# pandegroup/openmm

Hardware: NVIDIA H100
Metric: ns/day (higher is better)
Workload: dtype f32

## Files before the change

openmm_b200/csrc/engine.cu:

```cuda
#include "engine.h"
#include "../../include/b200md.h"
#include <stdexcept>
#include <algorithm>
#include <cmath>
#include <cstring>
#include <cstdlib>
#include <map>
#include <set>
#include <dlfcn.h>
#include <thread>

static std::string g_create_error;

template <class T> struct DevBuf {
    T* p = nullptr; size_t n = 0; bool owned = true;
    void attach(void* ptr, size_t count) { free(); p = (T*) ptr; n = count; owned = false; }
    void alloc(size_t count) {
        if (!owned) { if (count > n) throw std::runtime_error("window buffer too small"); return; }
        free(); n = count; if (count) CUDA_CHECK(cudaMalloc(&p, count*sizeof(T)));
    }
    void upload(const std::vector<T>& v) { if (v.size() > n) alloc(v.size()); if (!v.empty()) CUDA_CHECK(cudaMemcpy(p, v.data(), v.size()*sizeof(T), cudaMemcpyHostToDevice)); }
    void zero() { if (n) CUDA_CHECK(cudaMemset(p, 0, n*sizeof(T))); }
    void free() { if (p && owned) cudaFree(p); p = nullptr; n = 0; owned = true; }
    ~DevBuf() { free(); }
// ... 58 lines not shown
struct b200md_ctx {
    int device = 0;
    int natoms = 0, npad = 0, nblocks = 0;
    bool finalized = false;
    std::string err;
    cudaStream_t stream = nullptr;
    cudaStream_t streamPme = nullptr;
    cudaStream_t streamBonded = nullptr;
    cudaEvent_t evFork = nullptr, evJoin = nullptr, evJoinBonded = nullptr, evForkGrid = nullptr;
    bool pmeOnly = false;
    bool listDirty = true;
    bool overlapPme = true;
    bool pmeBrick = true;
    int brickAtoms = 64, brickPoints = 8192;
    bool listBuilt = false;
    std::vector<double> mass, charge, sigma, epsilon;
    b200md_nonbonded_desc nbdesc{};
    bool haveNb = false;
    struct { std::vector<int2> atoms; std::vector<double3> params; DevBuf<int2> atomsDev; DevBuf<double4> paramsDev; } exc;
    TermTable<int2, double2> bonds;
    TermTable<int4, double2> angles;
    TermTable<int4, double4> torsions;
    TermTable<int4, double> rb;
    CmapTable cmap;
    std::vector<int> conI, conJ; std::vector<double> conD;
    int cmFreq = 0;
    std::vector<int4> hUnitAtoms;
    double boxA[3] = {0, 0, 0}, boxB[3] = {0, 0, 0}, boxC[3] = {0, 0, 0};
    bool haveBox = false;
    bool haveOrigin = false;
    double padFrac = 0.10;
    DevBuf<float4> posq, velm, sposq[2], swrap[2], refPos, atomShift, blockCenter[2], blockHalf[2], superCenter[2], superHalf[2];
    DevBuf<float2> sigeps, ssigeps[2];
    DevBuf<double> chargeD; DevBuf<double2> sigepsD;
    DevBuf<long long> force;
    DevBuf<double> energy, cmScratch;
    DevBuf<int> molStart, molAtoms, cellOffset, sorig[2], sortedOf, cellRank, cellCount, cellFill, atomCell, tmpSorted, tileI[2], tileJ[2], tileMask[2], listCounters, counters, exclStart, exclList;
    DevBuf<unsigned int> maskPool[2];
    DevBuf<unsigned long long> stepCounter;
    DevBuf<unsigned int> blocksDone;
    bool stepStateValid = false;
    DevBuf<real> grid, eterm;
    DevBuf<long long> gridFixed;
    DevBuf<real2> cgrid;
    DevBuf<real2> tw[3];
    DevBuf<double> moduli[3];
    DevBuf<int4> unitAtoms; DevBuf<int> unitType; DevBuf<float4> unitParams;
    std::vector<int> ccmaCons;
    DevBuf<int> ccCompCon, ccCompAtom, ccRowStart, ccCol, ccAtoms, ccAStart, ccACon;
    DevBuf<int2> ccConAtoms; DevBuf<float> ccDist, ccRedMass, ccVal, ccDelta1, ccDelta2;
    DevBuf<float4> ccRij, ccXold, ccXunc;
    int precision = B200MD_PRECISION_SINGLE;
    DevBuf<float4> posqCorr; DevBuf<double4> velmD, unitParamsD;
    DevBuf<double> ccDistD, ccRedMassD, ccDelta1D, ccDelta2D; DevBuf<double4> ccRijD, ccXoldD, ccXuncD, ccXposD;
    bool mixed() const { return precision == B200MD_PRECISION_MIXED; }
    CcmaDev ccma{};
    NbDev nb{};
    PmeDev pme{};
    BondedDev bd{};
    UnitDev units{};
    IntegDev integ{};
    bool haveIntegrator = false;
    double dt = 0, temperature = 0, friction = 0;
    double time = 0;
    int64_t stepCount = 0;
    double selfEnergy = 0, dispersionCoefficient = 0;
    int64_t forceEvals = 0, kernelLaunches = 0, graphInstantiations = 0;
    DevBuf<int> baroStart, baroAtoms;
// ... 882 lines not shown
extern "C" int b200md_finalize(b200md_ctx* ctx) {
    API_BEGIN(ctx)
    require(!ctx->finalized, "finalize called twice");
    b200md_ctx* c = ctx;
    const int N = c->natoms, NP = c->npad;
    if (!c->haveNb) { c->nbdesc = b200md_nonbonded_desc{}; c->nbdesc.method = B200MD_NB_NOCUTOFF; }
    NbDev& nb = c->nb;
    nb.natoms = N; nb.npad = NP; nb.nblocks = c->nblocks;
    nb.method = c->nbdesc.method;
    nb.rank = c->rank; nb.world = c->world;
    c->cd = CommDev{}; c->cd.world = 1;
    c->p2p = c->world > 1 && c->comm && !(getenv("B200MD_MGPU") && std::string(getenv("B200MD_MGPU")) == "nccl");
    if (c->p2p) setup_window(c);
    { const double cc = getenv("B200MD_CLOSE_NM") ? atof(getenv("B200MD_CLOSE_NM")) : 0.36; nb.closeCut2 = (float) (cc*cc); }
    for (int w = 0; w < 4; w++) nb.pmeSmMask[w] = 0ull;
    nb.smPartition = false;
    if (c->nbdesc.method == B200MD_NB_PME && !c->pmeOnly && c->overlapPme) {
        int want = 0;
        if (c->p2p) want = std::min(74, std::max((c->nbdesc.grid[0] + c->world - 1)/c->world, 16 + 6*c->world));
        if (getenv("B200MD_PME_SMS")) want = atoi(getenv("B200MD_PME_SMS"));
        const int got = want > 0 ? choose_pme_sms(want, nb.pmeSmMask) : 0;
        if (got > 0) {
            nb.smPartition = true;
            const int planes = (c->nbdesc.grid[0] + c->world - 1)/c->world;
            fft_set_compact(planes > got ? 2 : 1);
        }
    }
    c->posq.alloc(NP); c->posq.zero(); c->velm.alloc(NP); c->velm.zero();
    c->refPos.alloc(NP); c->refPos.zero(); c->atomShift.alloc(NP); c->sigeps.alloc(NP);
    c->listCounters.alloc(2*LC_STRIDE); c->listCounters.zero();
    for (int l = 0; l < 2; l++) {
        c->sposq[l].alloc(NP); c->sposq[l].zero(); c->swrap[l].alloc(NP); c->swrap[l].zero(); c->ssigeps[l].alloc(NP); c->ssigeps[l].zero();
        c->sorig[l].alloc(NP); c->sorig[l].zero(); c->blockCenter[l].alloc(c->nblocks); c->blockHalf[l].alloc(c->nblocks);
        ListDev& L = c->nb.list[l];
        L.sposq = c->sposq[l].p; L.ssigeps = c->ssigeps[l].p; L.swrap = c->swrap[l].p; L.sorig = c->sorig[l].p;
        c->superCenter[l].alloc((c->nblocks + 31)/32); c->superHalf[l].alloc((c->nblocks + 31)/32);
        L.superCenter = c->superCenter[l].p; L.superHalf = c->superHalf[l].p;
        L.blockCenter = c->blockCenter[l].p; L.blockHalf = c->blockHalf[l].p; L.lc = c->listCounters.p + LC_STRIDE*l;
    }
    c->force.alloc((size_t) 3*NP); c->force.zero();
    c->energy.alloc(B200MD_NUM_ENERGY); c->energy.zero(); c->cmScratch.alloc(12); c->cmScratch.zero();
    c->blocksDone.alloc(1); c->blocksDone.zero();
    c->sortedOf.alloc(NP); c->atomCell.alloc(NP); c->tmpSorted.alloc(NP);
    c->counters.alloc(16); c->counters.zero();
    c->stepCounter.alloc(1); c->stepCounter.zero();
    std::vector<float4> vm(NP, make_float4(0, 0, 0, 0));
    for (int i = 0; i < N; i++) vm[i].w = (c->mass[i] > 0) ? (float) (1.0/c->mass[i]) : 0.f;
    c->velm.upload(vm);
    nb.posqCorr = nullptr; nb.velmD = nullptr;
    if (c->mixed()) {
        std::vector<double4> vd(NP, make_double4(0, 0, 0, 0));
        for (int i = 0; i < N; i++) vd[i].w = (c->mass[i] > 0) ? 1.0/c->mass[i] : 0.0;
        c->posqCorr.alloc(NP); c->posqCorr.zero(); c->velmD.upload(vd);
        nb.posqCorr = c->posqCorr.p; nb.velmD = c->velmD.p;
    }
    nb.posq = c->posq.p; nb.velm = c->velm.p; nb.sigeps = c->sigeps.p; nb.force = c->force.p; nb.energy = c->energy.p;
    nb.sortedOf = c->sortedOf.p;
    nb.refPos = c->refPos.p; nb.atomCell = c->atomCell.p; nb.tmpSorted = c->tmpSorted.p; nb.atomShift = c->atomShift.p;
    nb.counters = c->counters.p;
    const double rc = c->nbdesc.cutoff;
    if (nb.method == B200MD_NB_NOCUTOFF) {
        nb.cutoff = 1e18f; nb.cutoff2 = 3e38f; nb.paddedCutoff2 = 3e38f; nb.halfPad2 = 3e38f;
    }
    else {
        const double pad = c->padFrac*rc;
        nb.cutoff = (float) rc; nb.cutoff2 = (float) (rc*rc); nb.paddedCutoff2 = (float) ((rc+pad)*(rc+pad)); nb.halfPad2 = (float) (0.25*pad*pad);
    }
    nb.useSwitch = c->nbdesc.use_switch; nb.switchDist = (float) c->nbdesc.switch_distance;
    nb.alpha = (float) c->nbdesc.ewald_alpha;
    if (nb.method == B200MD_NB_CUTOFF_PERIODIC || nb.method == B200MD_NB_CUTOFF_NONPERIODIC) {
        const double eps = c->nbdesc.rf_dielectric;
        nb.krf = (float) (std::pow(rc, -3.0)*(eps-1.0)/(2.0*eps+1.0));
        nb.crf = (float) ((1.0/rc)*(3.0*eps)/(2.0*eps+1.0));
    }
    {
        std::vector<std::vector<int> > ex(N);
        for (const int2& a : c->exc.atoms) { ex[a.x].push_back(a.y); ex[a.y].push_back(a.x); }
        std::vector<int> start(N+1, 0), list;
        for (int i = 0; i < N; i++) {
            std::sort(ex[i].begin(), ex[i].end());
            ex[i].erase(std::unique(ex[i].begin(), ex[i].end()), ex[i].end());
            start[i+1] = start[i] + (int) ex[i].size();
            list.insert(list.end(), ex[i].begin(), ex[i].end());
        }
        if (list.empty()) list.push_back(0);
        c->exclStart.upload(start); c->exclList.upload(list);
        nb.exclStart = c->exclStart.p; nb.exclList = c->exclList.p;
    }
    alloc_tile_pools(c, initial_pool_capacity(c));
// ... 357 lines not shown
            launch_pme_spread(c->nb, pme, c->cd, sp, !forkAfterList); launches++;
            if (p2p) { launch_grid_push(c->pme, c->cd, sp); launches++; }
            else if (c->world > 1 && c->comm && !split) {
                int rc = g_nccl.AllReduce(c->gridFixed.p, c->gridFixed.p, (size_t) c->pme.nx*c->pme.ny*c->pme.nz, NCCL_INT64, NCCL_SUM, c->comm, sp);
                if (rc != 0) throw std::runtime_error("ncclAllReduce(grid) failed");
            }
            launch_pme_fft_conv(c->nb, c->pme, c->cd, energy && (split || p2p || c->rank == 0), fft_beside_tiles(c), sp); launches += pme_fft_launch_count(c->pme);
            launch_pme_gather(c->nb, pme, c->cd, sp); launches++;
        }
        if (fork) CUDA_CHECK(cudaEventRecord(c->evJoin, sp));
    };
    if (!forkAfterList) launch_recip();
    if (forkAfterList && recip) {
        CUDA_CHECK(cudaEventRecord(c->evForkGrid, s));
        CUDA_CHECK(cudaStreamWaitEvent(sp, c->evForkGrid, 0));
        CUDA_CHECK(cudaMemsetAsync(pme.gridFixed, 0, sizeof(long long)*(size_t) pme.nx*pme.ny*pme.nz, sp));
    }
    if (direct) {
        launch_check_displacement(c->nb, c->cd, s); launches++;
        launch_list_build(c->nb, s); launches += LIST_BUILD_LAUNCHES;
    }
    int bterms = terms & (B200MD_TERM_BONDS | B200MD_TERM_ANGLES | B200MD_TERM_TORSIONS | B200MD_TERM_RB_TORSIONS | B200MD_TERM_CMAP);
    if (c->haveNb) bterms |= terms & B200MD_TERM_NB_DIRECT;
    const int nbonded = c->bd.nbonds + c->bd.nangles + c->bd.ntorsions + c->bd.nrb + c->bd.ncmap + c->bd.nexc;
    const bool bonded = bterms && nbonded > 0 && !(split && c->rank == pmeRank);
    auto launch_bonded_terms = [&](cudaStream_t sb) { BondedDev bd = c->bd; bd.groupMask = groupMask; launch_bonded(c->nb, bd, bterms, energy, sb); launches++; };
    const bool forkBonded = forkAfterList && bonded;
    if (forkAfterList) launch_recip();
    if (forkBonded) {
        CUDA_CHECK(cudaStreamWaitEvent(c->streamBonded, c->evFork, 0));
        launch_bonded_terms(c->streamBonded);
        CUDA_CHECK(cudaEventRecord(c->evJoinBonded, c->streamBonded));
    }
    if (direct) { launch_pair(c->nb, energy, s); launches++; }
    if (bonded && !forkBonded) launch_bonded_terms(s);
    const bool pushEarly = p2p && fork;
    if (pushEarly) { launch_force_push(c->nb, c->cd, s); launches++; }
    if (fork) CUDA_CHECK(cudaStreamWaitEvent(s, c->evJoin, 0));
    if (forkBonded) CUDA_CHECK(cudaStreamWaitEvent(s, c->evJoinBonded, 0));
    if (p2p) {
        if (!pushEarly) { launch_force_push(c->nb, c->cd, s); launches++; }
        if (!inStep) { launch_force_total(c->nb, c->cd, s); launches += 2; }
    }
    if (c->world > 1 && c->comm) {
        int rc = 0;
        if (!p2p) rc = g_nccl.AllReduce(c->force.p, c->force.p, (size_t) 3*c->npad, NCCL_INT64, NCCL_SUM, c->comm, s);
        if (rc != 0) throw std::runtime_error("ncclAllReduce(force) failed");
        if (energy) {
            rc = g_nccl.AllReduce(c->energy.p, c->energy.p, B200MD_NUM_ENERGY, NCCL_FLOAT64, NCCL_SUM, c->comm, s);
            if (rc != 0) throw std::runtime_error("ncclAllReduce(energy) failed");
        }
    }
    CUDA_CHECK(cudaGetLastError());
    return launches;
}

static void check_flags(b200md_ctx* c) {
    if (!c->finalized) return;
    int h[8];
    CUDA_CHECK(cudaMemcpyAsync(h, c->counters.p, sizeof(int)*8, cudaMemcpyDeviceToHost, c->stream));
    CUDA_CHECK(cudaStreamSynchronize(c->stream));
    if (h[CT_OVERFLOW] == 2) throw std::runtime_error("B200 platform: neighbour-list construction timed out at a grid barrier (k_list_prep)");
    if (h[CT_OVERFLOW] == 3) throw std::runtime_error("B200 platform: multi-GPU exchange timed out waiting for a peer rank (every rank must issue the same sequence of calls)");
    if (h[CT_OVERFLOW]) throw std::runtime_error("B200 platform: neighbour-list tile capacity exceeded (" + std::to_string(c->nb.maxTiles) + " tiles) during the preceding steps; the trajectory since the last state read is invalid");
}

static bool role_split(const b200md_ctx* c);
// ... 404 lines not shown
```

openmm_b200/csrc/engine.h:

```cpp
#pragma once
#include <cuda_runtime.h>
#include <stdint.h>
#include <stdexcept>
#include <string>
#include <vector>

#define B200MD_TILE 32
#define B200MD_PME_ORDER 5
#define B200MD_FORCE_SCALE 4294967296.0
#define B200MD_ONE_4PI_EPS0 138.93545764438198
#define B200MD_BOLTZ 0.00831446261815324
#define B200MD_MAX_RADIX 16
#define B200MD_MAX_FFT_STAGES 8

#define CUDA_CHECK(x) do { cudaError_t e_ = (x); if (e_ != cudaSuccess) throw std::runtime_error(std::string(#x) + ": " + cudaGetErrorString(e_)); } while (0)

template <typename... P, typename... A>
inline void launch_high(void (*kernel)(P...), dim3 grid, dim3 block, size_t smem, cudaStream_t s, A... args) {
    static const int hi = [] { int lo = 0, h = 0; cudaDeviceGetStreamPriorityRange(&lo, &h); return h; }();
    cudaLaunchAttribute at[1];
    at[0].id = cudaLaunchAttributePriority;
    at[0].val.priority = hi;
    cudaLaunchConfig_t cfg = {};
    cfg.gridDim = grid; cfg.blockDim = block; cfg.dynamicSmemBytes = smem; cfg.stream = s;
    cfg.attrs = at; cfg.numAttrs = 1;
    CUDA_CHECK(cudaLaunchKernelEx(&cfg, kernel, args...));
}

struct BoxDev {
    float ax, bx, by, cx, cy, cz;
    float invAx, invBy, invCz;
    int triclinic;
    int periodic;
    double dax, dby, dcz;
    double recip[9];
    double volume;
};

#ifdef B200MD_REAL_DOUBLE
typedef double real;
typedef double2 real2;
#else
typedef float real;
typedef float2 real2;
#endif

struct FftPlanDev {
    int n;
    int nstages;
    int radix[B200MD_MAX_FFT_STAGES];
    const real2* tw;
};

struct ListDev {
    float4* sposq;
    float2* ssigeps;
    float4* swrap;
    int* sorig;
    float4* blockCenter;
    float4* blockHalf;
    float4* superCenter;
    float4* superHalf;
    int* tileI;
    int* tileJ;
    int* tileMask;
    unsigned int* maskPool;
    int* lc;
};
#define TILE_REGIONS 32
enum { LC_TILES = 0, LC_MASKS = TILE_REGIONS, LC_MAXHALF = 2*TILE_REGIONS, LC_USED = 2*TILE_REGIONS + 1, LC_STRIDE = 128 };

enum { CT_PAIRSTART = 0,
       CT_REBUILD = 2, CT_OVERFLOW = 3, CT_BUILDS = 4, CT_PAIRS = 5, CT_CUR = 10, CT_CURSOR = 14,
       CT_BTDONE = 7, CT_BAR = 9, CT_BAREXIT = 15 };

struct NbDev {
    BoxDev box;
    int natoms, npad, nblocks;
    int method;
    int useSwitch;
    float cutoff, cutoff2, paddedCutoff2, switchDist;
    float alpha;
    float krf, crf;
    float dispDummy;
    float4* posq;
    float4* velm;
    float4* posqCorr;
    double4* velmD;
    float2* sigeps;
    const double* chargeD;
    const double2* sigepsD;
    long long* force;
    double* energy;
    ListDev list[2];
    int* sortedOf;
    float4* refPos;
    int ncell[3];
    int ncells;
    const int* cellRank;
    int* cellCount;
    int* cellFill;
    int* atomCell;
    int* tmpSorted;
    float4* atomShift;
    int maxTiles;
    int* counters;
    const int* exclStart;
    const int* exclList;
    int nmol;
    const int* molStart;
    const int* molAtoms;
    int* cellOffset;
    float halfPad2;
    int rank, world;
    double origin[3];
    unsigned long long pmeSmMask[4];
    bool smPartition;
    float closeCut2;
};

enum { EN_NB = 0, EN_RECIP = 1, EN_BOND = 2, EN_ANGLE = 3, EN_TORSION = 4, EN_EXC = 5, EN_KE = 6, EN_RBTORSION = 7, EN_CMAP = 8,
       B200MD_NUM_ENERGY = 9 };

struct PmeDev {
    int nx, ny, nz, nzc;
// ... 215 lines not shown
        c = make_uint4(hi1 ^ c.y ^ k.x, lo1, hi0 ^ c.w ^ k.y, lo0);
        k.x += 0x9E3779B9u; k.y += 0xBB67AE85u;
    }
    return c;
}

__device__ __forceinline__ float3 gauss3(unsigned int seed, int atom, unsigned long long step) {
    uint4 r = philox(make_uint4((unsigned int) atom, (unsigned int) step, (unsigned int) (step >> 32), 0x5eed5eedu), make_uint2(seed, 0xb200b200u));
    const float u1 = ((r.x >> 8) + 1u)*(1.0f/16777216.0f);
    const float u2 = (r.y >> 8)*(1.0f/16777216.0f);
    const float u3 = ((r.z >> 8) + 1u)*(1.0f/16777216.0f);
    const float u4 = (r.w >> 8)*(1.0f/16777216.0f);
    const float m1 = sqrtf(-2.0f*logf(u1)), m2 = sqrtf(-2.0f*logf(u3));
    float s1, c1, s2, c2;
    sincospif(2.0f*u2, &s1, &c1);
    sincospif(2.0f*u4, &s2, &c2);
    (void) s2;
    return make_float3(m1*c1, m1*s1, m2*c2);
}

#endif

struct ScaleDev {
    int nmol;
    const int* molStart;
    const int* molAtoms;
    double a[3], b[3], c[3];
    double s[3];
};

void launch_check_displacement(const NbDev& nb, const CommDev& cd, cudaStream_t s);
const int LIST_BUILD_LAUNCHES = 2;
void launch_list_build(const NbDev& nb, cudaStream_t s);
void launch_pair(const NbDev& nb, bool energy, cudaStream_t s);
void pair_set_carveout(size_t fftSmem, size_t brickSmem);
void launch_count_pairs(const NbDev& nb, cudaStream_t s);
int choose_pme_sms(int reserve, unsigned long long mask[4]);

void launch_pme_eterm(const NbDev& nb, const PmeDev& pme, cudaStream_t s);
void launch_pme_spread(const NbDev& nb, const PmeDev& pme, const CommDev& cd, cudaStream_t s, bool zeroGrid = true);
void launch_pme_fft_conv(const NbDev& nb, const PmeDev& pme, const CommDev& cd, bool energy, bool besideTiles, cudaStream_t s);
void launch_pme_gather(const NbDev& nb, const PmeDev& pme, const CommDev& cd, cudaStream_t s);
void pme_brick_setup(int maxSmem);
void launch_grid_push(const PmeDev& pme, const CommDev& cd, cudaStream_t s);
void launch_fft3d_r2c(const PmeDev& pme, cudaStream_t s);
void launch_fft3d_c2r(const PmeDev& pme, cudaStream_t s);
size_t fft_plane_smem_bytes(int ny, int nz);
size_t fft_line_smem_bytes(int nx);
bool fft_make_radices(int n, int* radix, int* nstages);
int pme_fft_launch_count(const PmeDev& pme);
void fft_set_compact(int on);
size_t fft_cta_smem_bytes(const PmeDev& pme);
bool fft_slab_path(const PmeDev& pme);

void launch_bonded(const NbDev& nb, const BondedDev& bd, int terms, bool energy, cudaStream_t s);

void launch_integrate(const NbDev& nb, const UnitDev& units, const IntegDev& integ, const CommDev& cd, cudaStream_t s);
void launch_force_push(const NbDev& nb, const CommDev& cd, cudaStream_t s);
void launch_pos_push(const NbDev& nb, const CommDev& cd, const IntegDev& in, cudaStream_t s);
bool pos_push_available();
void launch_force_total(const NbDev& nb, const CommDev& cd, cudaStream_t s);
void launch_vel_push(const NbDev& nb, const CommDev& cd, cudaStream_t s);
void launch_pos_wait(const NbDev& nb, const CommDev& cd, cudaStream_t s);
void launch_constrain_positions(const NbDev& nb, const UnitDev& units, double tol, cudaStream_t s);
void launch_constrain_velocities(const NbDev& nb, const UnitDev& units, double tol, cudaStream_t s);
void launch_kinetic_energy(const NbDev& nb, const UnitDev& units, const IntegDev& integ, double shiftDt, cudaStream_t s);
// ... 7 lines not shown
```

openmm_b200/csrc/nonbonded.cu:

```cuda
#include "engine.h"
#include "../../include/b200md.h"
#include <algorithm>

#define FULL 0xffffffffu

__device__ __forceinline__ float3 min_image(float3 d, const BoxDev& b) {
    if (b.triclinic) {
        float s = floorf(d.z*b.invCz + 0.5f);
        d.x -= s*b.cx; d.y -= s*b.cy; d.z -= s*b.cz;
        s = floorf(d.y*b.invBy + 0.5f);
        d.x -= s*b.bx; d.y -= s*b.by;
        s = floorf(d.x*b.invAx + 0.5f);
        d.x -= s*b.ax;
    }
    else {
        d.x -= b.ax*rintf(d.x*b.invAx);
        d.y -= b.by*rintf(d.y*b.invBy);
        d.z -= b.cz*rintf(d.z*b.invCz);
    }
    return d;
}

__device__ __forceinline__ float box_dist2(float3 d, float hx, float hy, float hz, const BoxDev& b, bool periodic) {
    if (periodic) d = min_image(d, b);
// ... 118 lines not shown
    int run = partial[threadIdx.x] - sum;
    for (int i = begin; i < end; i++) {
        int c = nb.cellCount[i];
        nb.cellCount[i] = run;
        run += c;
    }
    if (threadIdx.x == 0) nb.cellCount[n] = nb.natoms;
}

__device__ __forceinline__ void fill_atom(const NbDev& nb, int a) {
    int key = nb.atomCell[a];
    int slot = nb.cellCount[key] + atomicAdd(&nb.cellFill[key], 1);
    nb.tmpSorted[slot] = a;
}

__device__ __forceinline__ void finalize_slot(const NbDev& nb, const ListDev& L, int s) {
    if (s < nb.natoms) {
        int a = s;
        if (nb.box.periodic) {
            a = nb.tmpSorted[s];
            const int key = nb.atomCell[a];
            const int begin = nb.cellCount[key], end = nb.cellCount[key+1];
            int rank = 0;
            for (int t = begin; t < end; t++) rank += (nb.tmpSorted[t] < a);
            s = begin + rank;
        }
        float4 p = nb.posq[a];
        float4 sh = nb.atomShift[a];
        L.sorig[s] = a;
        nb.sortedOf[a] = s;
        L.swrap[s] = make_float4(p.x+sh.x, p.y+sh.y, p.z+sh.z, p.w);
        L.sposq[s] = p;
        L.ssigeps[s] = nb.sigeps[a];
        nb.refPos[a] = p;
        if (s == 0) L.lc[LC_MAXHALF] = 0;
    }
    else {
        L.sorig[s] = -1;
        L.ssigeps[s] = make_float2(0, 0);
    }
}

__device__ __forceinline__ void grid_barrier(const NbDev& nb, int target) {
    __syncthreads();
    if (threadIdx.x == 0) {
        __threadfence();
        atomicAdd(&nb.counters[CT_BAR], 1);
        long spins = 0;
        while (*((volatile int*) &nb.counters[CT_BAR]) < target) {
            __nanosleep(32);
            if (++spins > (1L << 23)) { nb.counters[CT_OVERFLOW] = 2; break; }
        }
        __threadfence();
    }
    __syncthreads();
}

__device__ void list_prep_phases(const NbDev& nb, const ListDev& L, int* partial) {
    const int G = gridDim.x;
    const int gtid = blockIdx.x*blockDim.x + threadIdx.x, gthreads = G*blockDim.x;
    const int lane = threadIdx.x & 31, gwarp = gtid >> 5, gwarps = gthreads >> 5;
    int base = 0;
    if (nb.nmol > 0) {
        for (int m = gtid; m < nb.nmol; m += gthreads) wrap_molecule(nb, m);
        grid_barrier(nb, G);
        base = G;
    }
    for (int a = gtid; a < nb.natoms; a += gthreads) bin_atom(nb, a);
    grid_barrier(nb, base + G);
    if (blockIdx.x == 0) scan_cells_block(nb, partial);
    grid_barrier(nb, base + 2*G);
    for (int a = gtid; a < nb.natoms; a += gthreads) fill_atom(nb, a);
// ... 340 lines not shown
}

struct TileCursor {
    int incl, total, cap;
    __device__ __forceinline__ void init(const NbDev& nb, const ListDev& L, int lane) {
        cap = nb.maxTiles/TILE_REGIONS;
        int c = min(L.lc[LC_TILES + lane], cap);
        for (int off = 1; off < 32; off <<= 1) {
            const int v = __shfl_up_sync(FULL, c, off);
            if (lane >= off) c += v;
        }
        incl = c;
        total = __shfl_sync(FULL, c, 31);
    }
    __device__ __forceinline__ int slot(int f) const {
        const int r = __popc(__ballot_sync(FULL, incl <= f));
        const int before = __shfl_sync(FULL, incl, max(r-1, 0));
        return r*cap + f - (r > 0 ? before : 0);
    }
};
static_assert(TILE_REGIONS == 32, "TileCursor maps one pool to one lane");

__device__ __forceinline__ float wrap_rel(float p, float c, double L, double invL) {
    double r = (double) p - (double) c;
    r -= L*rint(r*invL);
    return (float) r;
}

#define CLOSE_QCAP 96
__device__ __forceinline__ float ewald_g(float w);
template <bool ENERGY, int METHOD, bool SWITCH>
__device__ __forceinline__ void close_pair_double(const NbDev& nb, const ListDev& L, int si, int sj, double& energyD) {
    const float4 a = L.sposq[si], b = L.sposq[sj];
    const int ai = L.sorig[si], aj = L.sorig[sj];
    const double qq = nb.chargeD[ai]*nb.chargeD[aj];
    const double2 sa = nb.sigepsD[ai], sb = nb.sigepsD[aj];
    double dx = (double) b.x - (double) a.x, dy = (double) b.y - (double) a.y, dz = (double) b.z - (double) a.z;
    const BoxDev& bx = nb.box;
    if (bx.periodic) {
        if (bx.triclinic) {
            double k = floor(dz*bx.recip[8] + 0.5);
            dx -= k*(double) bx.cx; dy -= k*(double) bx.cy; dz -= k*bx.dcz;
            k = floor(dy*bx.recip[4] + 0.5);
            dx -= k*(double) bx.bx; dy -= k*bx.dby;
            k = floor(dx*bx.recip[0] + 0.5);
            dx -= k*bx.dax;
        }
        else {
            dx -= bx.dax*rint(dx*bx.recip[0]); dy -= bx.dby*rint(dy*bx.recip[4]); dz -= bx.dcz*rint(dz*bx.recip[8]);
        }
    }
    const double r2 = dx*dx + dy*dy + dz*dz;
    const double invR = rsqrt(r2), invR2 = invR*invR;
    double dEdR, e = 0.0;
    if (METHOD == B200MD_NB_PME) {
        const float w = nb.alpha*nb.alpha*(float) r2;
        const double a3 = (double) nb.alpha*(double) nb.alpha*(double) nb.alpha;
        if (w < PME_G_WMAX && !ENERGY) dEdR = qq*(invR*invR2 - a3*(double) ewald_g(w));
        else {
            const double ar = (double) nb.alpha*r2*invR;
            const double ec = erfc(ar), ex = exp(-ar*ar);
            dEdR = qq*invR*invR2*(ec + 1.12837916709551257390*ar*ex);
            e = qq*invR*ec;
        }
    }
    else if (METHOD == B200MD_NB_NOCUTOFF) { dEdR = qq*invR*invR2; e = qq*invR; }
    else { dEdR = qq*(invR*invR2 - 2.0*(double) nb.krf); e = qq*(invR + (double) nb.krf*r2 - (double) nb.crf); }
    const double sig = sa.x + sb.x, eps = sa.y*sb.y;
    const double s2 = sig*sig*invR2, s6 = s2*s2*s2;
    double ljF = eps*s6*invR2*(12.0*s6 - 6.0), ljE = eps*s6*(s6 - 1.0);
    if (SWITCH) {
        const double r = r2*invR;
        if (r > (double) nb.switchDist) {
            const double swInv = 1.0/((double) nb.cutoff - (double) nb.switchDist);
            const double x = (r - (double) nb.switchDist)*swInv;
            const double sw = 1.0 + x*x*x*(-10.0 + x*(15.0 - x*6.0));
            const double dsw = x*x*(-30.0 + x*(60.0 - x*30.0))*swInv;
            ljF = sw*ljF - ljE*dsw*invR;
            ljE *= sw;
        }
    }
    dEdR += ljF;
    if (ENERGY) energyD += e + ljE;
    const long long fx = __double2ll_rn(dx*dEdR*B200MD_FORCE_SCALE), fy = __double2ll_rn(dy*dEdR*B200MD_FORCE_SCALE), fz = __double2ll_rn(dz*dEdR*B200MD_FORCE_SCALE);
    atomicAdd((unsigned long long*) &nb.force[ai], (unsigned long long) (-fx));
    atomicAdd((unsigned long long*) &nb.force[ai + nb.npad], (unsigned long long) (-fy));
    atomicAdd((unsigned long long*) &nb.force[ai + 2*nb.npad], (unsigned long long) (-fz));
    atomicAdd((unsigned long long*) &nb.force[aj], (unsigned long long) fx);
    atomicAdd((unsigned long long*) &nb.force[aj + nb.npad], (unsigned long long) fy);
    atomicAdd((unsigned long long*) &nb.force[aj + 2*nb.npad], (unsigned long long) fz);
}

template <bool ENERGY, int METHOD, bool SHIFT, bool SWITCH, bool CLOSE>
__device__ __forceinline__ void pair_tiles(const NbDev& nb, const ListDev& L, float& energy, unsigned short* cq) {
    const int lane = threadIdx.x & 31;
    const int gwarp = (blockIdx.x*blockDim.x + threadIdx.x) >> 5;
    const int nwarps = (gridDim.x*blockDim.x) >> 5;
    TileCursor cursor;
    cursor.init(nb, L, lane);
    const int ntiles = cursor.total;
    const bool periodic = nb.box.periodic != 0;
    const float cutoff2 = nb.cutoff2;
    const float swInv = SWITCH ? 1.0f/(nb.cutoff - nb.switchDist) : 0.f;
    const int srcIn = (lane & ~7) | ((lane + 1) & 7);
    const int srcOut = (lane + 8) & 31;
    const int sub = lane & 7;
    const float close2 = CLOSE ? nb.closeCut2 : 0.f;
    const unsigned int ltMask = (1u << lane) - 1u;
    double energyD = 0.0;
    __shared__ int sbase;
    int f = gwarp;
    const int wib = threadIdx.x >> 5, wpb = blockDim.x >> 5;
    if (nb.smPartition) f = ntiles;
    for (;; f += nwarps) {
        if (nb.smPartition) {
            __syncthreads();
            if (threadIdx.x == 0) sbase = atomicAdd(&nb.counters[CT_CURSOR], wpb);
            __syncthreads();
            f = sbase + wib;
            if (sbase >= ntiles) break;
            if (f >= ntiles) continue;
        }
        else if (f >= ntiles) break;
// ... 76 lines not shown
                if (r > nb.switchDist) {
                    const float x = (r - nb.switchDist)*swInv;
                    const float sw = 1.0f + x*x*x*(-10.0f + x*(15.0f - x*6.0f));
                    const float dsw = x*x*(-30.0f + x*(60.0f - x*30.0f))*swInv;
                    ljF = sw*ljF - ljE*dsw*y;
                    ljE *= sw;
                }
            }
            dEdR = valid ? dEdR + ljF : 0.f;
            if (ENERGY) energy += valid ? e + ljE : 0.f;
            fix = fmaf(-d.x, dEdR, fix); fiy = fmaf(-d.y, dEdR, fiy); fiz = fmaf(-d.z, dEdR, fiz);
            fjx = fmaf(d.x, dEdR, fjx); fjy = fmaf(d.y, dEdR, fjy); fjz = fmaf(d.z, dEdR, fjz);
            pj.x = __shfl_sync(FULL, pj.x, srcIn); pj.y = __shfl_sync(FULL, pj.y, srcIn);
            pj.z = __shfl_sync(FULL, pj.z, srcIn); pj.w = __shfl_sync(FULL, pj.w, srcIn);
            sej.x = __shfl_sync(FULL, sej.x, srcIn); sej.y = __shfl_sync(FULL, sej.y, srcIn);
            fjx = __shfl_sync(FULL, fjx, srcIn); fjy = __shfl_sync(FULL, fjy, srcIn); fjz = __shfl_sync(FULL, fjz, srcIn);
        }
        fiTx += fix; fiTy += fiy; fiTz += fiz;
        fjTx += fjx; fjTy += fjy; fjTz += fjz;
        pj.x = __shfl_sync(FULL, pj.x, srcOut); pj.y = __shfl_sync(FULL, pj.y, srcOut);
        pj.z = __shfl_sync(FULL, pj.z, srcOut); pj.w = __shfl_sync(FULL, pj.w, srcOut);
        sej.x = __shfl_sync(FULL, sej.x, srcOut); sej.y = __shfl_sync(FULL, sej.y, srcOut);
        fjTx = __shfl_sync(FULL, fjTx, srcOut); fjTy = __shfl_sync(FULL, fjTy, srcOut); fjTz = __shfl_sync(FULL, fjTz, srcOut);
        }

        if (CLOSE && qn > 0) {
            __syncwarp();
            for (int e = lane; e < qn; e += 32) {
                const int code = cq[e];
                close_pair_double<ENERGY, METHOD, SWITCH>(nb, L, ib*32 + (code & 31), L.tileJ[t*32 + (code >> 5)], energyD);
            }
            __syncwarp();
        }
        const int ai = L.sorig[si];
        if (ai >= 0) {
            atomicAdd((unsigned long long*) &nb.force[ai], (unsigned long long) float_to_fixed(fiTx));
            atomicAdd((unsigned long long*) &nb.force[ai + nb.npad], (unsigned long long) float_to_fixed(fiTy));
            atomicAdd((unsigned long long*) &nb.force[ai + 2*nb.npad], (unsigned long long) float_to_fixed(fiTz));
        }
        if (jidx >= 0) {
            const int aj = L.sorig[jidx];
            atomicAdd((unsigned long long*) &nb.force[aj], (unsigned long long) float_to_fixed(fjTx));
            atomicAdd((unsigned long long*) &nb.force[aj + nb.npad], (unsigned long long) float_to_fixed(fjTy));
            atomicAdd((unsigned long long*) &nb.force[aj + 2*nb.npad], (unsigned long long) float_to_fixed(fjTz));
        }
    }
    if (ENERGY && CLOSE && energyD != 0.0) atomicAdd(&nb.energy[EN_NB], energyD);
}

template <bool ENERGY, int METHOD, bool SHIFT>
__device__ __forceinline__ void pair_tiles_sw(const NbDev& nb, const ListDev& L, float& energy, unsigned short* cq) {
    if (nb.closeCut2 > 0.f) {
        if (nb.useSwitch) pair_tiles<ENERGY, METHOD, SHIFT, true, true>(nb, L, energy, cq);
        else pair_tiles<ENERGY, METHOD, SHIFT, false, true>(nb, L, energy, cq);
    }
    else {
        if (nb.useSwitch) pair_tiles<ENERGY, METHOD, SHIFT, true, false>(nb, L, energy, cq);
        else pair_tiles<ENERGY, METHOD, SHIFT, false, false>(nb, L, energy, cq);
    }
}

template <bool ENERGY, int METHOD>
__global__ void __launch_bounds__(256, ENERGY ? 2 : 4) k_pair(NbDev nb) {
    if (nb.smPartition) {
        unsigned int smid;
        asm("mov.u32 %0, %%smid;" : "=r"(smid));
        const bool reserved = (nb.pmeSmMask[(smid >> 6) & 3] >> (smid & 63)) & 1ull;
        if (threadIdx.x == 0) {
            atomicAdd(&nb.counters[CT_PAIRSTART], 1);
            if (reserved) {
                long spins = 0;
                while (*((volatile int*) &nb.counters[CT_PAIRSTART]) < (int) gridDim.x && ++spins < (1L << 20)) __nanosleep(200);
            }
        }
        if (reserved) { __syncthreads(); return; }
    }
    float energy = 0.f;
// ... 41 lines not shown
        CUDA_CHECK(cudaFuncSetAttribute(k, cudaFuncAttributePreferredSharedMemoryCarveout, percent));
    }
}

__global__ void k_smid_probe(unsigned long long* bitmap) {
    unsigned int smid;
    asm("mov.u32 %0, %%smid;" : "=r"(smid));
    if (threadIdx.x == 0) atomicOr(&bitmap[(smid >> 6) & 3], 1ull << (smid & 63));
    const long long t0 = clock64();
    while (clock64() - t0 < 20000) { }
}
int choose_pme_sms(int reserve, unsigned long long mask[4]) {
    mask[0] = mask[1] = mask[2] = mask[3] = 0ull;
    if (reserve <= 0) return 0;
    int dev = 0, sms = 132;
    cudaGetDevice(&dev);
    cudaDeviceGetAttribute(&sms, cudaDevAttrMultiProcessorCount, dev);
    unsigned long long* d = nullptr;
    unsigned long long h[4] = {0, 0, 0, 0};
    if (cudaMalloc(&d, sizeof(h)) != cudaSuccess) return 0;
    cudaMemset(d, 0, sizeof(h));
    k_smid_probe<<<sms*16, 128>>>(d);
    cudaMemcpy(h, d, sizeof(h), cudaMemcpyDeviceToHost);
    cudaFree(d);
    int found = 0, taken = 0;
    for (int w = 0; w < 4; w++) found += __builtin_popcountll(h[w]);
    if (found < sms) return 0;
    reserve = std::min(reserve, found/2);
    for (int id = 255; id >= 0 && taken < reserve; id--)
        if ((h[id >> 6] >> (id & 63)) & 1ull) { mask[id >> 6] |= 1ull << (id & 63); taken++; }
    return taken;
}

void launch_pair(const NbDev& nb, bool energy, cudaStream_t s) {
    if (energy) launch_pair_m<true>(nb, s); else launch_pair_m<false>(nb, s);
}

__global__ void k_count_pairs(NbDev nb) {
    const ListDev& L = nb.list[nb.counters[CT_CUR] & 1];
    const int lane = threadIdx.x & 31;
    const int gwarp = (blockIdx.x*blockDim.x + threadIdx.x) >> 5;
    const int nwarps = (gridDim.x*blockDim.x) >> 5;
    TileCursor cursor;
    cursor.init(nb, L, lane);
    const int ntiles = cursor.total;
    if (gwarp == 0 && lane == 0) L.lc[LC_USED] = ntiles;
    int count = 0;
    for (int f = gwarp; f < ntiles; f += nwarps) {
        const int t = cursor.slot(f);
        const int si = L.tileI[t]*32 + lane;
        const float4 pi = L.sposq[si];
        const int mi = L.tileMask[t];
        const unsigned int mask = (mi < 0) ? FULL : L.maskPool[mi*32 + lane];
        for (int k = 0; k < 32; k++) {
            int jidx = L.tileJ[t*32 + k];
            if (jidx < 0 || !((mask >> k) & 1u)) continue;
            float4 pj = L.sposq[jidx];
            float3 d = make_float3(pj.x-pi.x, pj.y-pi.y, pj.z-pi.z);
            if (nb.box.periodic) d = min_image(d, nb.box);
            if (d.x*d.x + d.y*d.y + d.z*d.z < nb.cutoff2) count++;
        }
    }
    for (int off = 16; off > 0; off >>= 1) count += __shfl_xor_sync(FULL, count, off);
    if (lane == 0 && count) atomicAdd(&nb.counters[CT_PAIRS], count);
}

void launch_count_pairs(const NbDev& nb, cudaStream_t s) {
    int dev = 0, sms = 132;
// ... 6 lines not shown
```

Before: 1423.

## Accumulate pair forces in sorted order and fold into atom order afterwards

The pair kernel now accumulates forces into a separate buffer indexed by sorted slot instead of scattering through sorig to original atom indices. A new fold kernel then adds each sorted slot's force into the original-order force array and clears the slot. Sorted double-precision charges and sigma/epsilon are also stored during the sort so close pairs avoid the indirect lookups. The aim is more coalesced, localized atomics and fewer gathers, at the cost of an extra kernel launch, extra memory traffic and extra buffers.

```diff
diff --git a/openmm_b200/csrc/engine.cu b/openmm_b200/csrc/engine.cu
--- a/openmm_b200/csrc/engine.cu
+++ b/openmm_b200/csrc/engine.cu
@@ -114,8 +114,8 @@
     double padFrac = 0.10;
     DevBuf<float4> posq, velm, sposq[2], swrap[2], refPos, atomShift, blockCenter[2], blockHalf[2], superCenter[2], superHalf[2];
     DevBuf<float2> sigeps, ssigeps[2];
-    DevBuf<double> chargeD; DevBuf<double2> sigepsD;
-    DevBuf<long long> force;
+    DevBuf<double> chargeD, schargeD[2]; DevBuf<double2> sigepsD, ssigepsD[2];
+    DevBuf<long long> force, forceS;
     DevBuf<double> energy, cmScratch;
     DevBuf<int> molStart, molAtoms, cellOffset, sorig[2], sortedOf, cellRank, cellCount, cellFill, atomCell, tmpSorted, tileI[2], tileJ[2], tileMask[2], listCounters, counters, exclStart, exclList;
     DevBuf<unsigned int> maskPool[2];
@@ -1064,13 +1064,15 @@
     for (int l = 0; l < 2; l++) {
         c->sposq[l].alloc(NP); c->sposq[l].zero(); c->swrap[l].alloc(NP); c->swrap[l].zero(); c->ssigeps[l].alloc(NP); c->ssigeps[l].zero();
         c->sorig[l].alloc(NP); c->sorig[l].zero(); c->blockCenter[l].alloc(c->nblocks); c->blockHalf[l].alloc(c->nblocks);
+        c->schargeD[l].alloc(NP); c->schargeD[l].zero(); c->ssigepsD[l].alloc(NP); c->ssigepsD[l].zero();
         ListDev& L = c->nb.list[l];
         L.sposq = c->sposq[l].p; L.ssigeps = c->ssigeps[l].p; L.swrap = c->swrap[l].p; L.sorig = c->sorig[l].p;
+        L.schargeD = c->schargeD[l].p; L.ssigepsD = c->ssigepsD[l].p;
         c->superCenter[l].alloc((c->nblocks + 31)/32); c->superHalf[l].alloc((c->nblocks + 31)/32);
         L.superCenter = c->superCenter[l].p; L.superHalf = c->superHalf[l].p;
         L.blockCenter = c->blockCenter[l].p; L.blockHalf = c->blockHalf[l].p; L.lc = c->listCounters.p + LC_STRIDE*l;
     }
-    c->force.alloc((size_t) 3*NP); c->force.zero();
+    c->force.alloc((size_t) 3*NP); c->force.zero(); c->forceS.alloc((size_t) 3*NP); c->forceS.zero();
     c->energy.alloc(B200MD_NUM_ENERGY); c->energy.zero(); c->cmScratch.alloc(12); c->cmScratch.zero();
     c->blocksDone.alloc(1); c->blocksDone.zero();
     c->sortedOf.alloc(NP); c->atomCell.alloc(NP); c->tmpSorted.alloc(NP);
@@ -1086,7 +1088,7 @@
         c->posqCorr.alloc(NP); c->posqCorr.zero(); c->velmD.upload(vd);
         nb.posqCorr = c->posqCorr.p; nb.velmD = c->velmD.p;
     }
-    nb.posq = c->posq.p; nb.velm = c->velm.p; nb.sigeps = c->sigeps.p; nb.force = c->force.p; nb.energy = c->energy.p;
+    nb.posq = c->posq.p; nb.velm = c->velm.p; nb.sigeps = c->sigeps.p; nb.force = c->force.p; nb.forceS = c->forceS.p; nb.energy = c->energy.p;
     nb.sortedOf = c->sortedOf.p;
     nb.refPos = c->refPos.p; nb.atomCell = c->atomCell.p; nb.tmpSorted = c->tmpSorted.p; nb.atomShift = c->atomShift.p;
     nb.counters = c->counters.p;
@@ -1510,7 +1512,7 @@
         launch_bonded_terms(c->streamBonded);
         CUDA_CHECK(cudaEventRecord(c->evJoinBonded, c->streamBonded));
     }
-    if (direct) { launch_pair(c->nb, energy, s); launches++; }
+    if (direct) { launch_pair(c->nb, energy, s); launches += PAIR_LAUNCHES; }
     if (bonded && !forkBonded) launch_bonded_terms(s);
     const bool pushEarly = p2p && fork;
     if (pushEarly) { launch_force_push(c->nb, c->cd, s); launches++; }
diff --git a/openmm_b200/csrc/engine.h b/openmm_b200/csrc/engine.h
--- a/openmm_b200/csrc/engine.h
+++ b/openmm_b200/csrc/engine.h
@@ -55,6 +55,8 @@
 struct ListDev {
     float4* sposq;
     float2* ssigeps;
+    double* schargeD;
+    double2* ssigepsD;
     float4* swrap;
     int* sorig;
     float4* blockCenter;
@@ -91,6 +93,7 @@
     const double* chargeD;
     const double2* sigepsD;
     long long* force;
+    long long* forceS;
     double* energy;
     ListDev list[2];
     int* sortedOf;
@@ -372,6 +375,7 @@
 void launch_check_displacement(const NbDev& nb, const CommDev& cd, cudaStream_t s);
 const int LIST_BUILD_LAUNCHES = 2;
 void launch_list_build(const NbDev& nb, cudaStream_t s);
+const int PAIR_LAUNCHES = 2;
 void launch_pair(const NbDev& nb, bool energy, cudaStream_t s);
 void pair_set_carveout(size_t fftSmem, size_t brickSmem);
 void launch_count_pairs(const NbDev& nb, cudaStream_t s);
diff --git a/openmm_b200/csrc/nonbonded.cu b/openmm_b200/csrc/nonbonded.cu
--- a/openmm_b200/csrc/nonbonded.cu
+++ b/openmm_b200/csrc/nonbonded.cu
@@ -174,12 +174,16 @@
         L.swrap[s] = make_float4(p.x+sh.x, p.y+sh.y, p.z+sh.z, p.w);
         L.sposq[s] = p;
         L.ssigeps[s] = nb.sigeps[a];
+        L.schargeD[s] = nb.chargeD[a];
+        L.ssigepsD[s] = nb.sigepsD[a];
         nb.refPos[a] = p;
         if (s == 0) L.lc[LC_MAXHALF] = 0;
     }
     else {
         L.sorig[s] = -1;
         L.ssigeps[s] = make_float2(0, 0);
+        L.schargeD[s] = 0.0;
+        L.ssigepsD[s] = make_double2(0.0, 0.0);
     }
 }
 
@@ -586,9 +590,8 @@
 template <bool ENERGY, int METHOD, bool SWITCH>
 __device__ __forceinline__ void close_pair_double(const NbDev& nb, const ListDev& L, int si, int sj, double& energyD) {
     const float4 a = L.sposq[si], b = L.sposq[sj];
-    const int ai = L.sorig[si], aj = L.sorig[sj];
-    const double qq = nb.chargeD[ai]*nb.chargeD[aj];
-    const double2 sa = nb.sigepsD[ai], sb = nb.sigepsD[aj];
+    const double qq = L.schargeD[si]*L.schargeD[sj];
+    const double2 sa = L.ssigepsD[si], sb = L.ssigepsD[sj];
     double dx = (double) b.x - (double) a.x, dy = (double) b.y - (double) a.y, dz = (double) b.z - (double) a.z;
     const BoxDev& bx = nb.box;
     if (bx.periodic) {
@@ -637,12 +640,12 @@
     dEdR += ljF;
     if (ENERGY) energyD += e + ljE;
     const long long fx = __double2ll_rn(dx*dEdR*B200MD_FORCE_SCALE), fy = __double2ll_rn(dy*dEdR*B200MD_FORCE_SCALE), fz = __double2ll_rn(dz*dEdR*B200MD_FORCE_SCALE);
-    atomicAdd((unsigned long long*) &nb.force[ai], (unsigned long long) (-fx));
-    atomicAdd((unsigned long long*) &nb.force[ai + nb.npad], (unsigned long long) (-fy));
-    atomicAdd((unsigned long long*) &nb.force[ai + 2*nb.npad], (unsigned long long) (-fz));
-    atomicAdd((unsigned long long*) &nb.force[aj], (unsigned long long) fx);
-    atomicAdd((unsigned long long*) &nb.force[aj + nb.npad], (unsigned long long) fy);
-    atomicAdd((unsigned long long*) &nb.force[aj + 2*nb.npad], (unsigned long long) fz);
+    atomicAdd((unsigned long long*) &nb.forceS[si], (unsigned long long) (-fx));
+    atomicAdd((unsigned long long*) &nb.forceS[si + nb.npad], (unsigned long long) (-fy));
+    atomicAdd((unsigned long long*) &nb.forceS[si + 2*nb.npad], (unsigned long long) (-fz));
+    atomicAdd((unsigned long long*) &nb.forceS[sj], (unsigned long long) fx);
+    atomicAdd((unsigned long long*) &nb.forceS[sj + nb.npad], (unsigned long long) fy);
+    atomicAdd((unsigned long long*) &nb.forceS[sj + 2*nb.npad], (unsigned long long) fz);
 }
 
 template <bool ENERGY, int METHOD, bool SHIFT, bool SWITCH, bool CLOSE>
@@ -785,17 +788,15 @@
             }
             __syncwarp();
         }
-        const int ai = L.sorig[si];
-        if (ai >= 0) {
-            atomicAdd((unsigned long long*) &nb.force[ai], (unsigned long long) float_to_fixed(fiTx));
-            atomicAdd((unsigned long long*) &nb.force[ai + nb.npad], (unsigned long long) float_to_fixed(fiTy));
-            atomicAdd((unsigned long long*) &nb.force[ai + 2*nb.npad], (unsigned long long) float_to_fixed(fiTz));
+        if (si < nb.natoms) {
+            atomicAdd((unsigned long long*) &nb.forceS[si], (unsigned long long) float_to_fixed(fiTx));
+            atomicAdd((unsigned long long*) &nb.forceS[si + nb.npad], (unsigned long long) float_to_fixed(fiTy));
+            atomicAdd((unsigned long long*) &nb.forceS[si + 2*nb.npad], (unsigned long long) float_to_fixed(fiTz));
         }
         if (jidx >= 0) {
-            const int aj = L.sorig[jidx];
-            atomicAdd((unsigned long long*) &nb.force[aj], (unsigned long long) float_to_fixed(fjTx));
-            atomicAdd((unsigned long long*) &nb.force[aj + nb.npad], (unsigned long long) float_to_fixed(fjTy));
-            atomicAdd((unsigned long long*) &nb.force[aj + 2*nb.npad], (unsigned long long) float_to_fixed(fjTz));
+            atomicAdd((unsigned long long*) &nb.forceS[jidx], (unsigned long long) float_to_fixed(fjTx));
+            atomicAdd((unsigned long long*) &nb.forceS[jidx + nb.npad], (unsigned long long) float_to_fixed(fjTy));
+            atomicAdd((unsigned long long*) &nb.forceS[jidx + 2*nb.npad], (unsigned long long) float_to_fixed(fjTz));
         }
     }
     if (ENERGY && CLOSE && energyD != 0.0) atomicAdd(&nb.energy[EN_NB], energyD);
@@ -903,8 +904,23 @@
     return taken;
 }
 
+__global__ void __launch_bounds__(256) k_fold_sorted(NbDev nb) {
+    const int s = blockIdx.x*blockDim.x + threadIdx.x;
+    if (s >= nb.natoms) return;
+    const ListDev& L = nb.list[nb.counters[CT_CUR] & 1];
+    const int a = L.sorig[s];
+    for (int c = 0; c < 3; c++) {
+        const long long v = nb.forceS[s + c*nb.npad];
+        if (v != 0) {
+            atomicAdd((unsigned long long*) &nb.force[a + c*nb.npad], (unsigned long long) v);
+            nb.forceS[s + c*nb.npad] = 0;
+        }
+    }
+}
+
 void launch_pair(const NbDev& nb, bool energy, cudaStream_t s) {
     if (energy) launch_pair_m<true>(nb, s); else launch_pair_m<false>(nb, s);
+    k_fold_sorted<<<(nb.natoms + 255)/256, 256, 0, s>>>(nb);
 }
 
 __global__ void k_count_pairs(NbDev nb) {
```

Measured after the change: 1473, median of 6. 3.5% higher.
